# ilia-glushchenko/SimplePathTracer

Measured on AMD Instinct MI355X. Metric: Msamples/s (pixels×spp/s), RTIOW random-sphere scene, 1/2/4/8 MI355X, higher is better.
Workload: dtype f32

## Files before the change

simplepathtracer_amd/csrc/spt_kernels.hip:

```cpp
#include "spt_path.h"
#include "spt_decode.h"

#include <algorithm>
#include <mutex>

namespace spt {


#ifndef SPT_WAVES_PER_EU
#define SPT_WAVES_PER_EU 0
#endif
#ifndef SPT_NUM_SGPR
#define SPT_NUM_SGPR 96
#endif
#if SPT_WAVES_PER_EU
#define SPT_RENDER_ATTR __attribute__((amdgpu_waves_per_eu(SPT_WAVES_PER_EU, SPT_WAVES_PER_EU)))
#elif SPT_NUM_SGPR
#define SPT_CAP_WAVES (800 / (((SPT_NUM_SGPR - 2 + 15) / 16) * 16 + 16) > 8 ? 8 : 800 / (((SPT_NUM_SGPR - 2 + 15) / 16) * 16 + 16))
#define SPT_RENDER_ATTR __attribute__((amdgpu_num_sgpr(SPT_NUM_SGPR), amdgpu_waves_per_eu(SPT_CAP_WAVES)))
#else
#define SPT_RENDER_ATTR
#endif

#ifndef SPT_LDS_BLOCK
// ... 308 lines not shown
                    acc.z = acc.z + c[i].z;
                    if constexpr (!TAB) acc.w = acc.w + 1.f;
                }
            }
            if constexpr (TAB) acc.w = acc.w + (float)kFoldRun;
        }
        for (; k < S; ++k) {
            uint32_t w;
            if constexpr (TAB) {
                w = *ps;
                ps += stp;
            } else {
                w = samples[q0 + k * step];
            }
            const f3 c = decode_word<TAB>(a, w);
            acc.x = acc.x + c.x;
            acc.y = acc.y + c.y;
            acc.z = acc.z + c.z;
            acc.w = acc.w + 1.f;
        }
    } else if (!alias) {
        const uint2 *s2 = (const uint2 *)samples;
        for (uint32_t k = 0; k < S; ++k) {
            const uint2 v = s2[q0 + k * step];
            if (v.y != 0u) {
                const f3 c = decode_word<TAB>(a, v.x);
                acc.x = acc.x + c.x;
                acc.y = acc.y + c.y;
                acc.z = acc.z + c.z;
                acc.w = acc.w + 1.f;
            }
        }
    } else {
        alias_accumulate<TAB>(a, samples, p, W, rows, 0u, rows, S, acc);
    }
    if (!a.last) {
        a.acc[p] = acc;
        if (!a.preview) return;
    }
    const float scale = a.mode == 0 ? 1.f / (float)a.s_done : 1.f / acc.w;
    const float r = acc.x * scale, g = acc.y * scale, b = acc.z * scale;
    if (out_rgba) out_rgba[p] = make_float4(r, g, b, 0.f);
    if (out_rgb8) {
        const uint32_t x = map.x0 + col;
        const uint32_t y = row_of(map, lr);
        const size_t gi = (size_t)3 * ((size_t)(a.height - 1u - y) * a.width + x);
        out_rgb8[gi + 0] = gamma_byte(r);
        out_rgb8[gi + 1] = gamma_byte(g);
        out_rgb8[gi + 2] = gamma_byte(b);
    }
}

#ifndef SPT_SVC_WT
#define SPT_SVC_WT 1
#endif

__device__ __forceinline__ void svc_flush(uint32_t idx, uint32_t cnt, uint32_t lane)
{
    if (cnt == 0u) return;
    kargs_t &k = *kernarg_args();
    asm volatile("s_waitcnt vmcnt(0)" ::: "memory");
    if (!SPT_SVC_WT) {
        __builtin_amdgcn_fence(__ATOMIC_RELEASE, "agent");
        asm volatile("s_waitcnt vmcnt(0)" ::: "memory");
    }
    if (lane == 0) __hip_atomic_fetch_add((gu32 *)(k.svc_done + idx), cnt, __ATOMIC_RELAXED, __HIP_MEMORY_SCOPE_AGENT);
    if (k.svc_trace && lane == 0) atomicMax(k.svc_trace + 4u * idx + 2u, __builtin_amdgcn_s_memrealtime());
}

template <bool TREE, int LEAF, bool LDSN, uint32_t BLOCK, bool BATCH = false, bool GLANE = false, bool SVC = false>
__device__ __forceinline__ void render_body(const RenderArgs &a)
{
    static_assert(!SVC || (!GLANE && !BATCH && (LDSN || SPT_PRIM)),
                  "the render service runs the wave-walk kernel or the LDS lane walk");
    const uint32_t lane = __lane_id();
    const uint32_t rows = SVC ? 0u : a.npix / a.map.width;

    __shared__ uint32_t s_lds[BLOCK];
    __shared__ uint4 s_nodes[LDSN ? 2 * (SVC ? kLdsSvcNodeRecords : kLdsNodeRecords) : 1];
    constexpr bool LDS_BYTES = LDSN && SPT_LANE_WALK && SPT_LANE_BUDGET > 0;
    constexpr bool PRIM = SPT_PRIM && !LDSN && !GLANE;
    constexpr uint32_t PW = kParkWords + (SVC ? 1u : 0u);
    __shared__ uint32_t s_park[PRIM ? (BLOCK / 64u) * PW * 64u : 1];
    uint32_t *const park = s_park + (PRIM ? opaque_v((threadIdx.x >> 6) * PW * 64u + lane) : 0u);
    auto prow = [&](uint32_t r) -> int32_t { return (int32_t)r - (int32_t)lane; };
    __shared__ uint32_t s_rec[SVC ? (BLOCK / 64u) * kSvcRecWords : 1];
    uint32_t *const rec = s_rec + (SVC ? (threadIdx.x >> 6) * kSvcRecWords : 0u);
    if (SVC && lane < kSvcRecWords - kSvcSt) rec[kSvcSt + lane] = 0u;
    if (SVC && !LDSN && blockIdx.x == 0u && (threadIdx.x >> 6) == 0u) {
        svc_forward(lane);
        return;
    }
    uint32_t q_n = 0, q_pos = 0;
    if (LDSN) {
        const uint4 *src = (const uint4 *)a.scene.accel.nodes;
        const uint32_t n4 = 2u * (a.scene.accel.n_nodes + 1u);
        for (uint32_t k = threadIdx.x; k < n4; k += BLOCK) {
            uint4 v = src[k];
            if (LDS_BYTES && (k & 1u)) v.x <<= 5;
            s_nodes[k] = v;
        }
        __syncthreads();
        if (SVC && blockIdx.x == 0u && (threadIdx.x >> 6) == 0u) {
            svc_forward(lane);
            return;
        }
    }
    Path ps;
    ps.phase = PH_IDLE;
    ps.item = ps.bounce = ps.spec = 0;
    ps.st = 0;
    ps.o = ps.d = mk(0.f, 0.f, 0.f);
    ps.slot = 0;
    ps.job = 0;

    uint32_t blk_cur = 0, blk_end = 0;
    uint32_t pend = 0;
    uint32_t rect = 0;
    const uint32_t home = blockIdx.x % a.n_queues;
    uint32_t qi = 0;
    if (SVC)
        pend = svc_reserve(home, lane, 0u);
    else if (lane == 0)
        pend = claim_next(a, home, qi);
    bool exhausted = false;
    uint32_t acc_idx = 0, acc_cnt = 0;
    unsigned long long casts = 0, done = 0, dropped = 0;
    struct {
        unsigned long long iters = 0, cast = 0, shade = 0, refill = 0;
        unsigned long long p_iters = 0, p_nodes = 0, p_spheres = 0, p_branches = 0, p_cast = 0;
        unsigned long long s_rounds[3] = {0, 0, 0};
        unsigned long long t_iters = 0, t_live = 0;
    } dc;
    CastDiag dg;
    Hit hres;
    hres.idx = kMiss;
    hres.best = FLT_MAX;
    hres.t = 0.f;
    uint32_t li = 0, lleaf = kNoSlot, lleaf2 = kNoSlot;
    bool fresh = true;
#if SPT_DIAG
    unsigned long long d_t0 = __builtin_amdgcn_s_memtime();
#define SPT_STAMP(acc)                                              \
    do {                                                            \
        const unsigned long long t_ = __builtin_amdgcn_s_memtime(); \
        acc += t_ - d_t0;                                           \
        d_t0 = t_;                                                  \
    } while (0)
#else
#define SPT_STAMP(acc) \
    do {               \
    } while (0)
#endif

    auto take_items = [&](unsigned long long need) -> uint32_t {
        const uint32_t cnt = (uint32_t)__popcll(need);
        const uint32_t rank = lane_rank(need);
        const uint32_t avail = blk_end - blk_cur;
        uint32_t mine = 0xFFFFFFFFu;
        if (rank < avail) mine = blk_cur + rank;
        if (avail >= cnt) {
            blk_cur += cnt;
        } else {
            const uint32_t nb = __builtin_amdgcn_readfirstlane(pend);
            if (nb < a.n_items && lane == 0) pend = claim_next(a, home, qi);
            if (nb >= a.n_items) {
                exhausted = true;
                blk_cur = blk_end = 0;
            } else {
                const uint32_t ne = min(nb + a.claim, a.n_items);
                const uint32_t r2 = rank - avail;
                if (rank >= avail && r2 < ne - nb) mine = nb + r2;
                blk_cur = nb + min(cnt - avail, ne - nb);
                blk_end = ne;
            }
        }
        return __builtin_amdgcn_inverse_ballot_w64(need) ? mine : 0xFFFFFFFFu;
    };

    auto next_claim = [&]() {
        const uint32_t nb = __builtin_amdgcn_readfirstlane(pend);
        if (nb < a.n_items && lane == 0) pend = claim_next(a, home, qi);
        if (nb >= a.n_items) {
            exhausted = true;
        } else {
            blk_cur = nb;
            blk_end = min(nb + a.claim, a.n_items);
            rect = find_rect(nb);
        }
    };

    auto next_claim_svc = [&]() {
        uint32_t *const st = rec + kSvcSt;
        const uint32_t nb = __builtin_amdgcn_readfirstlane(pend) * a.n_queues + home;
        uint32_t pc = __builtin_amdgcn_readfirstlane(st[0]);
        if (nb >= pc) {
            const unsigned long long p = svc_pub();
            pc = __builtin_amdgcn_readfirstlane((uint32_t)p);
            const uint32_t pj = __builtin_amdgcn_readfirstlane((uint32_t)(p >> 32));
            if (lane == 0) {
                st[0] = pc;
                st[1] = pj;
            }
        }
        exhausted = nb >= pc;
        if (exhausted) return;
        pend = svc_reserve(home, lane, pend);
        if (nb >= __builtin_amdgcn_readfirstlane(st[3])) {
            const uint32_t cur = svc_find_job(nb, __builtin_amdgcn_readfirstlane(st[2]),
                                              __builtin_amdgcn_readfirstlane(st[1]), rec, lane);
            const uint32_t ce = __builtin_amdgcn_readfirstlane(rec[7]);
            if (lane == 0) {
                st[2] = cur;
                st[3] = ce;
            }
        }
        blk_cur = nb * a.claim;
        blk_end = min(blk_cur + a.claim, __builtin_amdgcn_readfirstlane(rec[1]));
        kargs_t &kt = *kernarg_args();
        if (kt.svc_trace && lane == 0) {
            const unsigned long long t = __builtin_amdgcn_s_memrealtime();
            unsigned long long *tr = kt.svc_trace + 4u * rec[3];
            atomicMin(tr, t);
            atomicMax(tr + 1, t);
            if (nb < kSvcTraceClaims)
                kt.svc_trace[4u * 4096u + nb] = (t & 0xFFFFFFFFFFull) | ((unsigned long long)blockIdx.x << 40);
        }
    };

    for (;;) {
        unsigned long long need = __ballot(ps.phase == PH_IDLE);
        if (__popcll(need) < (PRIM ? SPT_PRIM_REFILL_MIN : SPT_REFILL_MIN) && need != ~0ull) need = 0ull;
        bool prim_iter = false;
        uint32_t pxy = 0;
        if (PRIM) {
            if (need != 0ull) {
                const uint32_t cnt = (uint32_t)__popcll(need);
                const uint32_t rank = lane_rank(need);
                const uint32_t take = min(cnt, q_n - q_pos);
                if (ps.phase == PH_IDLE && rank < take) unpark_path<SVC>(park, prow(q_pos + rank), ps);
                q_pos += take;
                bool more = !exhausted;
                if (SVC && cnt > take) {
                    if (blk_cur == blk_end) next_claim_svc();
                    more = blk_cur < blk_end;
                }
                if (cnt > take && more) {
                    park_path<SVC>(park, 0, ps);
                    asm volatile("" ::: "memory");
                    ps.phase = PH_IDLE;
                    if (SVC) {
                        const uint32_t n = min(64u, blk_end - blk_cur);
                        const uint32_t mine = blk_cur + lane;
                        blk_cur += n;
                        if (lane < n) start_path_svc(mine, rec, ps, &pxy);
                    } else if (BATCH) {
                        if (blk_cur == blk_end) next_claim();
                        if (!exhausted) {
                            const uint32_t n = min(64u, blk_end - blk_cur);
                            const uint32_t mine = blk_cur + lane;
                            blk_cur += n;
                            if (lane < n) start_path_rect(mine, rect, ps, &pxy);
                        }
                    } else {
                        const uint32_t mine = take_items(~0ull);
                        if (mine != 0xFFFFFFFFu) start_path_kernarg(mine, rows, ps, &pxy);
                        if ((SPT_DUP & 4) && mine != 0xFFFFFFFFu) {
                            Path p2;
                            uint32_t pxy2 = 0;
                            start_path_kernarg(opaque_v(mine), rows, p2, &pxy2);
                            sink_v(p2.d.x);
                            sink_v(p2.d.y);
                            sink_v(p2.d.z);
                            sink_v(p2.st);
                            sink_v(pxy2);
                        }
                    }
                    prim_iter = true;
                }
            }
        } else if (SVC && !PRIM && need != 0ull) {
            if (blk_cur == blk_end) next_claim_svc();
            if (blk_cur < blk_end) {
                const uint32_t take = min((uint32_t)__popcll(need), blk_end - blk_cur);
                const uint32_t rank = lane_rank(need);
                if (__builtin_amdgcn_inverse_ballot_w64(need) && rank < take) start_path_svc(blk_cur + rank, rec, ps);
                blk_cur += take;
            }
        } else if (BATCH && need != 0ull && !exhausted) {
            if (blk_cur == blk_end) next_claim();
            if (!exhausted) {
                const uint32_t take = min((uint32_t)__popcll(need), blk_end - blk_cur);
                const uint32_t rank = lane_rank(need);
                const uint32_t mine = blk_cur + rank;
                blk_cur += take;
                if (ps.phase == PH_IDLE && rank < take) {
                    start_path_rect(mine, rect, ps);
                }
            }
        } else if (!BATCH && need != 0ull && !exhausted) {
            const uint32_t mine = take_items(need);
            if (mine != 0xFFFFFFFFu) start_path_kernarg(mine, rows, ps);
        }
        const unsigned long long live = __ballot(ps.phase != PH_IDLE);
        if (live == 0ull) {
            if (PRIM && prim_iter) {
                unpark_path<SVC>(park, 0, ps);
                q_n = q_pos = 0;
                continue;
            }
            if (SVC && q_pos == q_n) {
                svc_flush(acc_idx, acc_cnt, lane);
                acc_cnt = 0;
                unsigned long long t0 = __builtin_amdgcn_s_memrealtime();
                bool leave = false;
                bool closing = false;
                uint32_t committed = 0;
                for (;;) {
                    const bool stop = svc_stopped();
                    if (stop) {
                        asm volatile("s_waitcnt vmcnt(0)" ::: "memory");
                        __builtin_amdgcn_fence(__ATOMIC_ACQUIRE, "agent");
                    }
                    if (closing) {
                        kargs_t &k = *kernarg_args();
                        const uint32_t c = lane == 0 ? __hip_atomic_load((gu32 *)(k.svc_host + kSvcHostCommitted),
                                                                         __ATOMIC_SEQ_CST, __HIP_MEMORY_SCOPE_SYSTEM)
                                                     : 0u;
                        asm volatile("s_waitcnt vmcnt(0)" ::: "memory");
                        __builtin_amdgcn_fence(__ATOMIC_ACQUIRE, "agent");
                        committed = __builtin_amdgcn_readfirstlane(c);
                    }
                    next_claim_svc();
                    if (!exhausted) break;
                    if (stop) {
                        leave = true;
                        break;
                    }
                    if (closing) {
                        if (__builtin_amdgcn_readfirstlane(rec[kSvcSt + 1]) >= committed) {
                            kargs_t &k = *kernarg_args();
                            if (lane == 0)
                                __hip_atomic_store((gu32 *)(k.svc_host + kSvcHostWatchdog), 1u, __ATOMIC_RELAXED,
                                                   __HIP_MEMORY_SCOPE_SYSTEM);
                            leave = true;
                            break;
                        }
                        closing = false;
                        t0 = __builtin_amdgcn_s_memrealtime();
                    } else if (__builtin_amdgcn_s_memrealtime() - t0 > kSvcIdleTicks) {
                        kargs_t &k = *kernarg_args();
                        if (lane == 0)
                            __hip_atomic_store((gu32 *)(k.svc_host + kSvcHostClosing), 1u, __ATOMIC_SEQ_CST,
                                               __HIP_MEMORY_SCOPE_SYSTEM);
                        asm volatile("s_waitcnt vmcnt(0)" ::: "memory");
                        __builtin_amdgcn_fence(__ATOMIC_SEQ_CST, "");
                        closing = true;
                        continue;
                    }
                    __builtin_amdgcn_s_sleep(8);
                }
                if (leave) break;
                continue;
            }
            if (exhausted && q_pos == q_n) break;
            continue;
        }
        SPT_STAMP(dc.refill);
#if SPT_DIAG
        const unsigned long long d_n0 = dg.nodes, d_s0 = dg.spheres, d_b0 = dg.branches, d_c0 = dc.cast;
#endif
        constexpr bool RES = SPT_LANE_BUDGET > 0 && (LDSN || GLANE);
        if (!RES) casts += (unsigned long long)__popcll(live);
        ++dc.iters;
        if (SPT_DIAG && exhausted) {
            dc.t_iters += 1;
            dc.t_live += (unsigned long long)__popcll(live);
        }
        const bool act = ps.phase != PH_IDLE;
        bool cdone = true;
        Hit h;
        if constexpr (RES) {
            if (SPT_DUP & 512) {
                Hit h2 = hres;
                h2.best = opaque_v(h2.best);
                uint32_t li2 = opaque_v(li), ll2 = lleaf, ll22 = lleaf2;
                const bool c2 = lane_cast<LEAF, LDS_BYTES>(a.scene.accel, opaque_v3(ps.o), opaque_v3(ps.d), act, dg,
                                    LDSN ? (const uint32_t *)s_nodes : (const uint32_t *)a.scene.accel.nodes, fresh,
                                    (uint32_t)SPT_LANE_BUDGET, h2, li2, ll2, ll22);
                sink_v(h2.idx);
                sink_v(h2.best);
                sink_v(li2);
                sink_v(c2 ? 1u : 0u);
            }
            cdone = lane_cast<LEAF, LDS_BYTES>(a.scene.accel, ps.o, ps.d, act, dg,
                                    LDSN ? (const uint32_t *)s_nodes : (const uint32_t *)a.scene.accel.nodes, fresh,
                                    (uint32_t)SPT_LANE_BUDGET, hres, li, lleaf, lleaf2);
            h = hres;
            casts += (unsigned long long)__popcll(__ballot(act && cdone));
        } else if constexpr (PRIM) {
            bool listed = false;
            if (prim_iter && kernarg_args()->prim.on) {
                if (SPT_DUP & 64) {
                    Hit h2;
                    prim_list_cast(a.scene.accel, opaque_v3(ps.o), opaque_v3(ps.d), act, pxy, h2, dg);
                    sink_v(h2.idx);
                    sink_v(h2.best);
                    sink_v(h2.t);
                }
                listed = prim_list_cast(a.scene.accel, ps.o, ps.d, act, pxy, h, dg);
            }
            if (!listed)
                h = find_closest<TREE, LEAF, LDSN>(a.scene.accel, ps.o, ps.d, act, dg, (const uint32_t *)s_nodes,
                                                   s_lds + (threadIdx.x & ~63u));
            if (SPT_DUP & 1) {
                const f3 o2 = opaque_v3(ps.o), d2 = opaque_v3(ps.d);
                Hit h2;
                bool l2 = false;
                if (prim_iter && kernarg_args()->prim.on) l2 = prim_list_cast(a.scene.accel, o2, d2, act, pxy, h2, dg);
                if (!l2) h2 = find_closest<TREE, LEAF, LDSN>(a.scene.accel, o2, d2, act, dg, (const uint32_t *)s_nodes);
                sink_v(h2.idx);
                sink_v(h2.best);
                sink_v(h2.t);
            }
        } else {
            h = (LDSN && SPT_LANE_WALK)
                    ? find_closest_lane<LEAF>(a.scene.accel, ps.o, ps.d, act, dg, (const uint32_t *)s_nodes)
                : GLANE
                    ? find_closest_lane<LEAF>(a.scene.accel, ps.o, ps.d, act, dg, (const uint32_t *)a.scene.accel.nodes)
                    : find_closest<TREE, LEAF, LDSN>(a.scene.accel, ps.o, ps.d, act, dg, (const uint32_t *)s_nodes);
        }
        SPT_STAMP(dc.cast);
#if SPT_DIAG
        if (prim_iter) {
            dc.p_iters += 1;
            dc.p_nodes += dg.nodes - d_n0;
            dc.p_spheres += dg.spheres - d_s0;
            dc.p_branches += dg.branches - d_b0;
            dc.p_cast += dc.cast - d_c0;
        }
#endif
        shade_step<true, SVC && SPT_SVC_WT>(a, ps, h, act && cdone, done, dropped, s_lds + (threadIdx.x & ~63u),
                                            SPT_DIAG ? dc.s_rounds : nullptr);
        fresh = cdone;
        if (SVC) {
            const bool fin = act && ps.phase == PH_IDLE;
            unsigned long long fm = __ballot(fin);
            while (fm != 0ull) {
                const uint32_t j = __builtin_amdgcn_readlane(ps.job, (int)__builtin_ctzll(fm));
                const unsigned long long m = __ballot(fin && ps.job == j);
                if (j != acc_idx) {
                    svc_flush(acc_idx, acc_cnt, lane);
                    acc_idx = j;
                    acc_cnt = 0;
                }
                acc_cnt += (uint32_t)__popcll(m);
                fm &= ~m;
            }
        }
        if (PRIM && prim_iter) {
            Path own;
            unpark_path<SVC>(park, 0, own);
            __builtin_amdgcn_wave_barrier();
            const unsigned long long lv = __ballot(ps.phase != PH_IDLE);
            if (ps.phase != PH_IDLE) park_path<SVC>(park, prow(lane_rank(lv)), ps);
            ps = own;
            q_n = (uint32_t)__popcll(lv);
            q_pos = 0;
        }
        SPT_STAMP(dc.shade);
    }

    if (SVC) {
        svc_flush(acc_idx, acc_cnt, lane);
        kargs_t &k = *kernarg_args();
        if (lane == 0) __hip_atomic_fetch_add((gu32 *)(k.svc_ctl + kSvcLive), 0xFFFFFFFFu, __ATOMIC_RELAXED, __HIP_MEMORY_SCOPE_AGENT);
    }
#pragma unroll
    for (int o = 32; o > 0; o >>= 1) {
        done += __shfl_xor(done, o);
        dropped += __shfl_xor(dropped, o);
    }
    if (lane == 0) {
        if (casts) atomicAdd(&a.counters[0], casts);
        if (done) atomicAdd(&a.counters[1], done);
        if (dropped) atomicAdd(&a.counters[2], dropped);
    }
#if SPT_DIAG
    if (lane == 0) {
        atomicAdd(&a.counters[4], dc.iters);
        atomicAdd(&a.counters[5], dg.leaves);
        atomicAdd(&a.counters[6], dg.nodes);
        atomicAdd(&a.counters[7], dc.cast);
        atomicAdd(&a.counters[8], dc.shade);
        atomicAdd(&a.counters[9], dc.refill);
        atomicAdd(&a.counters[10], dg.pairs);
        atomicAdd(&a.counters[11], dg.live);
        atomicAdd(&a.counters[12], dg.spheres);
        atomicAdd(&a.counters[13], dg.branches);
        atomicAdd(&a.counters[14], dg.passing);
        atomicAdd(&a.counters[15], dg.improving);
        atomicAdd(&a.counters[16], dg.lane_tests);
        atomicAdd(&a.counters[17], dg.lane_pretests);
        atomicAdd(&a.counters[18], dc.p_iters);
        atomicAdd(&a.counters[19], dc.p_nodes);
        atomicAdd(&a.counters[20], dc.p_spheres);
        atomicAdd(&a.counters[21], dc.p_branches);
        atomicAdd(&a.counters[22], dc.p_cast);
        atomicAdd(&a.counters[23], dc.s_rounds[0]);
        atomicAdd(&a.counters[24], dc.s_rounds[1]);
        atomicAdd(&a.counters[25], dg.leaves8);
        atomicAdd(&a.counters[26], dg.leaves16);
        atomicAdd(&a.counters[27], dc.s_rounds[2]);
        atomicAdd(&a.counters[28], dc.t_iters);
        atomicAdd(&a.counters[29], dc.t_live);
    }
#endif
#undef SPT_STAMP
}

template <bool TREE, int LEAF>
__global__ __launch_bounds__(kRenderBlock) SPT_RENDER_ATTR void render_kernel(RenderArgs a)
{
    render_body<TREE, LEAF, false, kRenderBlock>(a);
}

template <bool TREE, int LEAF>
__global__ __launch_bounds__(kRenderBlock) SPT_RENDER_ATTR void render_kernel_batch(RenderArgs a)
{
    render_body<TREE, LEAF, false, kRenderBlock, true>(a);
}

template <bool TREE, int LEAF>
__global__ __launch_bounds__(kRenderBlock) SPT_RENDER_ATTR void render_kernel_svc(RenderArgs a)
{
    render_body<TREE, LEAF, false, kRenderBlock, false, false, true>(a);
}

__global__ __launch_bounds__(kRenderBlock) SPT_RENDER_ATTR void render_kernel_glane(RenderArgs a)
{
    render_body<true, (int)kClusterSlots, false, kRenderBlock, false, true>(a);
}
__global__ __launch_bounds__(kRenderBlock) SPT_RENDER_ATTR void render_kernel_glane_batch(RenderArgs a)
{
    render_body<true, (int)kClusterSlots, false, kRenderBlock, true, true>(a);
}

#ifndef SPT_LDS_NUM_SGPR
#define SPT_LDS_NUM_SGPR 80
#endif
__global__ __launch_bounds__(kLdsBlock)
    __attribute__((amdgpu_num_sgpr(SPT_LDS_NUM_SGPR), amdgpu_waves_per_eu(2 * kLdsBlock / 256))) void render_kernel_lds(RenderArgs a)
{
    render_body<true, (int)kClusterSlots, true, kLdsBlock>(a);
}
__global__ __launch_bounds__(kLdsBlock)
    __attribute__((amdgpu_num_sgpr(SPT_LDS_NUM_SGPR), amdgpu_waves_per_eu(2 * kLdsBlock / 256))) void render_kernel_lds_batch(RenderArgs a)
{
    render_body<true, (int)kClusterSlots, true, kLdsBlock, true>(a);
}

__global__ __launch_bounds__(kLdsBlock)
    __attribute__((amdgpu_num_sgpr(SPT_LDS_NUM_SGPR), amdgpu_waves_per_eu(2 * kLdsBlock / 256))) void render_kernel_svc_lds(RenderArgs a)
{
    render_body<true, (int)kClusterSlots, true, kLdsBlock, false, false, true>(a);
}

#ifndef SPT_FOLD_PRIO
#define SPT_FOLD_PRIO 3
#endif
// ... 298 lines not shown
```

simplepathtracer_amd/csrc/spt_path.h:

```cpp
#pragma once
#include "spt_device.h"
#include "spt_internal.h"

#include <float.h>

#ifndef SPT_GROUP
#define SPT_GROUP 4
#endif

#ifndef SPT_DIAG
#define SPT_DIAG 0
#endif
#ifndef SPT_LEAF_SPLIT
#define SPT_LEAF_SPLIT 1
#endif
#ifndef SPT_DUP
#define SPT_DUP 0
#endif
#ifndef SPT_SAMPLER_SKIP0
#define SPT_SAMPLER_SKIP0 1
#endif
#ifndef SPT_SAMPLER_EVEN
#define SPT_SAMPLER_EVEN 1
#endif
// ... 909 lines not shown
    const uint32_t bw = k.prim.bw;
    const uint32_t x = pxy & 0xFFFFu, y = pxy >> 16;
    const float dod = dot(o, d);
    cfloat *slots = (cfloat *)ac.slots;
    cuint *ids = (cuint *)k.prim.slots;
    if (SPT_DIAG) dg.live_now = (uint32_t)__popcll(live);
    auto test_run = [&](uint2 e) {
        for (uint32_t i = e.x; i < e.x + e.y; i += 4u) {
            uint32_t s[4];
            float4 sp[4];
#pragma unroll
            for (int q = 0; q < 4; ++q) s[q] = ids[i + q];
#pragma unroll
            for (int q = 0; q < 4; ++q) sp[q] = ld_uniform(slots, s[q]);
            float tcv[4], hv[4];
            bool pass[4];
#pragma unroll
            for (int q = 0; q < 4; ++q) pass[q] = ray_sphere(sp[q], o, d, tcv[q], hv[q]);
            if (SPT_DIAG) dg.lane_tests += 4ull * dg.live_now;
#pragma unroll
            for (int q = 0; q < 4; ++q) {
                const unsigned long long pm = __ballot(pass[q]);
                if (SPT_DIAG) {
                    dg.spheres += 1;
                    dg.branches += pm != 0ull ? 1 : 0;
                }
                if (pm != 0ull) update_member(pm, tcv[q], hv[q], ac.orig, s[q], o, d, dod, h, dg);
            }
        }
    };
    const uint32_t b8 = (y >> 3) * bw + (x >> 3);
    const uint32_t lead = __builtin_amdgcn_readlane(b8, (int)__builtin_ctzll(live));
    if (__ballot(active && b8 != lead) == 0ull) {
        cuint *blk = (cuint *)k.prim.b8 + 2u * lead;
        const uint2 e = make_uint2(blk[0], blk[1]);
        if (e.y == kPrimWalk) return false;
        test_run(e);
        return true;
    }
    const uint32_t b4 = (y >> 2) * bw + (x >> 3);
    unsigned long long todo = live;
    while (todo != 0ull) {
        const uint32_t b = __builtin_amdgcn_readlane(b4, (int)__builtin_ctzll(todo));
        cuint *blk = (cuint *)k.prim.b4 + 2u * b;
        const uint2 e = make_uint2(blk[0], blk[1]);
        if (e.y == kPrimWalk) return false;
        test_run(e);
        todo &= ~__ballot(active && b4 == b);
    }
    return true;
}

__device__ __forceinline__ void refract_event(const float4 *__restrict__ slots, Path &ps, uint32_t idx)
{
    const float4 cs = slots[idx];
    const f3 C = mk(cs.x, cs.y, cs.z);
    const f3 nrm = normalize(sub(ps.o, C));
    const f3 d = ps.d;
    const float cc = dot(neg(nrm), d);
    f3 nd;
    if (uniform(ps.st, 0.f, 1.f) < schlick(kRsq, cc)) {
        nd = reflect(d, nrm);
    } else if (no_tir(kAirToGlass, cc)) {
        const f3 d2 = refract_dir(d, nrm, kAirToGlass, cc);
        const f3 rs = sub(C, ps.o);
        const float tc = dot(rs, d2);
        const float dd = lensq(rs) - tc * tc;
        const float t = tc + __builtin_sqrtf(cs.w - dd);
        ps.o = mk(ps.o.x + d2.x * t, ps.o.y + d2.y * t, ps.o.z + d2.z * t);
        const f3 n2 = neg(normalize(sub(ps.o, C)));
        const float c2 = dot(neg(n2), d2);
        if (uniform(ps.st, 0.f, 1.f) < schlick(kRsq, c2))
            nd = reflect(d2, n2);
        else if (no_tir(kGlassToAir, c2))
            nd = refract_dir(d2, n2, kGlassToAir, c2);
        else
            nd = reflect(d2, n2);
    } else {
        nd = reflect(d, nrm);
    }
    ps.d = nd;
}

template <bool WT = false>
__device__ __forceinline__ void finish_step(uint32_t mode, uint32_t *samples, Path &ps, unsigned long long finm,
                                            unsigned long long specm, unsigned long long refrm, unsigned long long skym,
                                            uint32_t word, unsigned long long &done, unsigned long long &dropped)
{
    typedef __attribute__((address_space(1))) uint32_t gu32_t;
    typedef __attribute__((address_space(1))) unsigned long long gu64_t;
    const uint32_t k = ps.spec & 0xFFFFu;
    const bool spec_event = __builtin_amdgcn_inverse_ballot_w64(specm);
    if (mode == 0u) {
        ps.spec += spec_event ? 1u : 0u;
        const unsigned long long capm = specm & __ballot(k + 1u > kSpecularCap);
        word = __builtin_amdgcn_inverse_ballot_w64(capm) ? kZeroWord : word;
        if (__builtin_amdgcn_inverse_ballot_w64(finm | capm)) {
            if (WT)
                __hip_atomic_store((gu32_t *)(samples + ps.item), word, __ATOMIC_RELAXED, __HIP_MEMORY_SCOPE_AGENT);
            else
                samples[ps.item] = word;
            ps.phase = PH_IDLE;
            ps.d = mk(0.f, 0.f, 0.f);
            ++done;
        }
        return;
    }
    bool fin = __builtin_amdgcn_inverse_ballot_w64(finm);
    const bool refr_event = __builtin_amdgcn_inverse_ballot_w64(refrm), sky = __builtin_amdgcn_inverse_ballot_w64(skym);
    bool counted = true;
    if (spec_event) {
        if (mode == 1u && k < kTaskPasses && refr_event) ps.spec |= 1u << (16u + k);
        ++ps.spec;
        if (mode == 1u && k + 1u >= kTaskPasses) {
            fin = true;
            counted = false;
            word = kZeroWord;
            ++dropped;
        } else if (k + 1u > kSpecularCap) {
            fin = true;
            word = kZeroWord;
        }
    }
    if (fin) {
        const uint32_t key =
            counted ? 1u + (((ps.spec & 0xFFFFu) << 11) | (sky ? 1u << 10 : 0u) | ((ps.spec >> 16) & 0x3FFu)) : 0u;
        if (WT)
            __hip_atomic_store((gu64_t *)(samples + (size_t)2 * ps.item), (unsigned long long)word | ((unsigned long long)key << 32),
                               __ATOMIC_RELAXED, __HIP_MEMORY_SCOPE_AGENT);
        else
            *(uint2 *)(samples + (size_t)2 * ps.item) = make_uint2(word, key);
        ps.phase = PH_IDLE;
        ps.d = mk(0.f, 0.f, 0.f);
        ++done;
    }
}

template <bool KARG, bool WT, bool SAMPLER>
__device__ __forceinline__ void shade_step_body(const RenderArgs &a, Path &ps, const Hit &h, bool act,
                                                unsigned long long &done, unsigned long long &dropped, uint32_t *lds,
                                                unsigned long long *diag_rounds)
{
    const float4 *__restrict__ hit = a.scene.accel.slots;
    const float4 *__restrict__ shade = a.scene.shade;
    const uint32_t *__restrict__ mat = a.scene.mat;
    uint32_t *samples = a.samples;
    uint32_t mode = a.mode;
    uint32_t bounces = a.bounces, code_stride = a.scene.code_stride, code_jmax = a.scene.code_jmax;
    if constexpr (KARG) {
        kargs_t &k = *kernarg_args();
        hit = k.scene.accel.slots;
        shade = k.scene.shade;
        mat = k.scene.mat;
        samples = k.samples;
        mode = k.mode;
        bounces = k.bounces;
        code_stride = k.scene.code_stride;
        code_jmax = k.scene.code_jmax;
    }
    const uint32_t idx = h.idx;
    const unsigned long long actm = __ballot(act);
    const unsigned long long hitm = actm & __ballot(idx != kMiss);
    uint32_t m = SPT_SKYBOX_ID;
    if (__builtin_amdgcn_inverse_ballot_w64(hitm)) m = mat[idx];
    const unsigned long long dlm = actm & __ballot(ps.phase == PH_DLOOP);
    const bool dl = __builtin_amdgcn_inverse_ballot_w64(dlm);
    const uint32_t nb = ps.bounce - 1u;
    ps.bounce = dl ? nb : ps.bounce;
    const unsigned long long endm = dlm & (__ballot(nb == 0u) | ~hitm);
    const unsigned long long trm = actm & ~dlm;
    const unsigned long long diffm = trm & __ballot(m == SPT_DIFFUSE_ID);
    const unsigned long long mirm = trm & __ballot(m == SPT_REFLECTIVE_ID);
    const unsigned long long refrm = trm & __ballot(m == SPT_REFRACTIVE_ID);
    const unsigned long long skym = trm & ~(diffm | mirm | refrm);
    const unsigned long long scatm = (dlm & ~endm) | diffm | mirm;
    const uint32_t j = min(bounces - nb - 1u, code_jmax);
    uint32_t word = kZeroWord;
    word = __builtin_amdgcn_inverse_ballot_w64(endm) ? code_word(diffuse_code(j, ps.slot, code_stride)) : word;
    word = __builtin_amdgcn_inverse_ballot_w64(skym) ? __float_as_uint(ps.d.y + 1.f) : word;
    const f3 rv_coop = SAMPLER ? coop_ball_vector(ps.st, scatm, lds, diag_rounds) : opaque_v3(mk(0.1f, 0.2f, 0.3f));
    if ((SPT_DUP & 2) && SAMPLER) {
        uint64_t st2 = opaque_v(ps.st);
        const bool scatter = __builtin_amdgcn_inverse_ballot_w64(scatm);
        const f3 r2 = coop_ball_vector(st2, __ballot(opaque_v(scatter ? 1u : 0u) != 0u), lds);
        sink_v(r2.x);
        sink_v(r2.y);
        sink_v(r2.z);
        sink_v(st2);
    }
    if (__builtin_amdgcn_inverse_ballot_w64(scatm)) {
        const float4 cs = hit[idx];
        const f3 C = mk(cs.x, cs.y, cs.z);
        ps.o = contact(ps.o, ps.d, h.t);
        const f3 nrm = normalize(sub(ps.o, C));
        f3 rv = rv_coop;
        const f3 on = add(ps.o, nrm);
        f3 base = mk(dl ? on.x : nrm.x, dl ? on.y : nrm.y, dl ? on.z : nrm.z);
        if (__builtin_amdgcn_inverse_ballot_w64(mirm)) {
            base = reflect(ps.d, nrm);
            rv = mul(rv, shade[idx].w);
        }
        ps.d = normalize(add(base, rv));
    }
    const bool first = __builtin_amdgcn_inverse_ballot_w64(diffm);
    ps.slot = first ? idx : ps.slot;
    ps.phase = first ? PH_DLOOP : ps.phase;
    if (__builtin_amdgcn_inverse_ballot_w64(refrm)) {
        ps.o = contact(ps.o, ps.d, h.t);
        if (SPT_DUP & 256) {
            Path p2 = ps;
            p2.o = opaque_v3(p2.o);
            refract_event(hit, p2, idx);
            sink_v(p2.d.x);
            sink_v(p2.o.x);
            sink_v(p2.st);
        }
        refract_event(hit, ps, idx);
    }
    finish_step<WT>(mode, samples, ps, endm | skym, mirm | refrm, refrm, trm, word, done, dropped);
}
template <bool KARG = false, bool WT = false>
__device__ __forceinline__ void shade_step(const RenderArgs &a, Path &ps, const Hit &h, bool act,
                                           unsigned long long &done, unsigned long long &dropped, uint32_t *lds,
                                           unsigned long long *diag_rounds = nullptr)
{
    if (SPT_DUP & 128) {
        Path p2 = ps;
        p2.o = opaque_v3(p2.o);
        p2.d = opaque_v3(p2.d);
        Hit h2 = h;
        h2.t = opaque_v(h2.t);
        unsigned long long d2 = 0, x2 = 0;
        shade_step_body<KARG, WT, false>(a, p2, h2, act, d2, x2, lds, nullptr);
        sink_v(p2.o.x);
        sink_v(p2.d.x);
        sink_v(p2.st);
    }
    shade_step_body<KARG, WT, true>(a, ps, h, act, done, dropped, lds, diag_rounds);
}



__device__ __forceinline__ void start_path(const RenderArgs &a, uint32_t mine, uint32_t rows, const Recip &rw,
                                           const Recip &rh, const f3 &eye, Path &ps, uint32_t *pxy = nullptr)
{
    uint32_t sl, lr, cx;
    ts_item(mine, a.map.width, rows, a.spp_batch, a.div_band, a.div_tile, sl, lr, cx);
    const uint32_t s = a.s0 + sl;
    ps.item = mine;
    const uint32_t x = a.map.x0 + cx;
    const uint32_t y = a.map.parts == 1u ? a.map.y0 + lr : row_of_fast(a.map, lr, a.div_strip);
    if (pxy) *pxy = (y << 16) | x;
    ps.st = fmix64(a.seed_key ^ (((uint64_t)(y * a.width + x) << 32) | (uint64_t)s));
    const float un = (float)y + uniform(ps.st, -1.f, 1.f);
    const float vn = (float)x + uniform(ps.st, -1.f, 1.f);
    float u = div_core(un, rw), v = div_core(vn, rh);
    if (__builtin_expect(!(div_operand_ok(un) && div_operand_ok(vn)), 0)) {
        u = un / (float)a.width;
        v = vn / (float)a.height;
    }
    const float vx = -1.f + 2.f * v, vy = -1.f + 2.f * u;
    const float *m = a.cam.view;
    ps.d = normalize(mk((m[0] * vx + m[1] * vy) + (m[2] * 1.f + m[3] * 0.f),
                        (m[4] * vx + m[5] * vy) + (m[6] * 1.f + m[7] * 0.f),
                        (m[8] * vx + m[9] * vy) + (m[10] * 1.f + m[11] * 0.f)));
    ps.o = eye;
    ps.phase = PH_TRACE;
    ps.bounce = a.bounces;
    ps.spec = 0;
}

__device__ __forceinline__ void start_path_kernarg(uint32_t mine, uint32_t rows, Path &ps, uint32_t *pxy = nullptr)
{
    kargs_t &k = *kernarg_args();
    RenderArgs a;
    a.map = RowMap{k.map.y0, k.map.y1, k.map.strip, k.map.parts, k.map.part, k.map.x0, k.map.width};
    a.width = k.width;
    a.height = k.height;
    a.bounces = k.bounces;
    a.npix = k.npix;
    a.n_items = k.n_items;
    a.spp_batch = k.spp_batch;
    a.s0 = k.s0;
    a.seed_key = k.seed_key;
    a.div_band = FastDiv{k.div_band.d, k.div_band.m, k.div_band.s};
    a.div_tile = FastDiv{k.div_tile.d, k.div_tile.m, k.div_tile.s};
    a.div_strip = FastDiv{k.div_strip.d, k.div_strip.m, k.div_strip.s};
#pragma unroll
    for (int q = 0; q < 12; ++q) a.cam.view[q] = k.cam.view[q];
    start_path(a, mine, rows, recip((float)a.width), recip((float)a.height),
               mk(k.cam.eye[0], k.cam.eye[1], k.cam.eye[2]), ps, pxy);
}

typedef __attribute__((address_space(4))) const BatchRect crect_t;
__device__ __forceinline__ uint32_t find_rect(uint32_t nb)
{
    kargs_t &k = *kernarg_args();
    crect_t *r = k.inline_rects ? (crect_t *)k.rects_inline : (crect_t *)k.rects;
    uint32_t lo = 0, hi = k.n_rects;
    while (hi - lo > 1u) {
        const uint32_t mid = (lo + hi) >> 1;
        if (r[mid].item_off <= nb) lo = mid; else hi = mid;
    }
    return lo;
}

__device__ __forceinline__ void start_path_rect(uint32_t mine, uint32_t ri, Path &ps, uint32_t *pxy = nullptr)
{
    kargs_t &k = *kernarg_args();
    crect_t &r = (k.inline_rects ? (crect_t *)k.rects_inline : (crect_t *)k.rects)[ri];
    if (mine >= r.item_end) return;
    RenderArgs a;
    a.map = RowMap{r.y0, r.y0 + r.rows, 1u, 1u, 0u, r.x0, r.w};
    a.width = k.width;
    a.height = k.height;
// ... 42 lines not shown
```

simplepathtracer_amd/csrc/spt_trace.hip:

```cpp
#include "spt_query.h"
#include "spt_decode.h"

namespace spt {

namespace {

constexpr uint32_t kTraceLaunchRays = 1u << 28;

template <bool TREE, int LEAF, int WALK, uint32_t BLOCK>
__device__ __forceinline__ void trace_body(const TraceArgs &a)
{
    constexpr bool AHEAD = WALK != kWalkLds;
    __shared__ uint32_t s_lds[BLOCK];
    const AccelView &ac = a.scene.accel;
    const uint32_t *const nodes = lds_node_table<WALK, BLOCK>(ac);
    RenderArgs ra;
    ra.scene = a.scene;
    ra.bounces = a.bounces;
    ra.mode = 0u;
    ra.samples = (uint32_t *)a.rgba;
    uint32_t *const lds = s_lds + (threadIdx.x & ~63u);

    const uint32_t lane = __lane_id();
    const uint32_t wave = __builtin_amdgcn_readfirstlane(blockIdx.x * (BLOCK / 64u) + (threadIdx.x >> 6));
    const uint32_t n_waves = gridDim.x * (BLOCK / 64u);
    const uint32_t runs = (a.n + 63u) >> 6;
    uint32_t run = wave, q_n = 0, q_pos = 0;
    f3 qo = mk(0.f, 0.f, 0.f), qd = mk(0.f, 0.f, 0.f);
    uint32_t qs_lo = 0, qs_hi = 0;
    auto load_run = [&]() {
        q_n = run < runs ? min(64u, a.n - (run << 6)) : 0u;
        q_pos = 0;
        if (AHEAD && lane < q_n) {
            const uint32_t i = (run << 6) + lane;
            const float4 o4 = a.o[i], d4 = a.d[i];
            const uint64_t st = a.st[i];
            qo = mk(o4.x, o4.y, o4.z);
            qd = mk(d4.x, d4.y, d4.z);
            qs_lo = (uint32_t)st;
            qs_hi = (uint32_t)(st >> 32);
        }
    };
    load_run();

    Path ps;
    ps.phase = PH_IDLE;
    ps.item = ps.bounce = ps.spec = 0;
    ps.st = 0;
    ps.o = ps.d = mk(0.f, 0.f, 0.f);
    ps.slot = 0;
    ps.job = 0;
    uint32_t casts = 0;
    unsigned long long done = 0, dropped = 0;
    CastDiag dg;

    for (;;) {
        const unsigned long long need = __ballot(ps.phase == PH_IDLE);
        if (need != 0ull && q_n != 0u) {
            const uint32_t take = min((uint32_t)__popcll(need), q_n - q_pos);
            const uint32_t rank = lane_rank(need);
            const bool get = __builtin_amdgcn_inverse_ballot_w64(need) && rank < take;
            const int from = (int)(get ? q_pos + rank : lane);
            f3 o = mk(0.f, 0.f, 0.f), d = o;
            uint64_t st = 0;
            if (AHEAD) {
                o = mk(__shfl(qo.x, from), __shfl(qo.y, from), __shfl(qo.z, from));
                d = mk(__shfl(qd.x, from), __shfl(qd.y, from), __shfl(qd.z, from));
                st = ((uint64_t)(uint32_t)__shfl((int)qs_hi, from) << 32) | (uint32_t)__shfl((int)qs_lo, from);
            }
            if (get) {
                const uint32_t i = (run << 6) + (uint32_t)from;
                if (!AHEAD) {
                    const float4 o4 = a.o[i], d4 = a.d[i];
                    st = a.st[i];
                    o = mk(o4.x, o4.y, o4.z);
                    d = mk(d4.x, d4.y, d4.z);
                }
                ps.o = o;
                ps.d = d;
                ps.st = st;
                ps.item = 4u * i;
                ps.phase = PH_TRACE;
                ps.bounce = a.bounces;
                ps.spec = 0;
                casts = 0;
            }
            q_pos += take;
            if (q_pos == q_n) {
                run += n_waves;
                load_run();
            }
        }
        const unsigned long long live = __ballot(ps.phase != PH_IDLE);
        if (live == 0ull) {
            if (q_n == 0u) break;
            continue;
        }
        const bool act = ps.phase != PH_IDLE;
        const Hit h = query_cast<TREE, LEAF, WALK>(ac, ps.o, ps.d, act, dg, nodes, lds);
        casts += act ? 1u : 0u;
        shade_step(ra, ps, h, act, done, dropped, lds);
        if (act && ps.phase == PH_IDLE && a.info) {
            const uint32_t ev = ps.spec & 0xFFFFu;
            uint32_t *rec = a.info + (ps.item >> 1);
            rec[0] = casts;
            rec[1] = ev | (ev > kSpecularCap ? 0x80000000u : 0u);
        }
    }
}

constexpr uint32_t kTraceBlock = 256, kTraceLdsBlock = 1024;

}

template <bool TREE, int LEAF>
__global__ __launch_bounds__(kTraceBlock) __attribute__((amdgpu_waves_per_eu(6))) void trace_kernel(TraceArgs a)
{
    trace_body<TREE, LEAF, kWalkWave, kTraceBlock>(a);
}
__global__ __launch_bounds__(kTraceBlock) void trace_kernel_glane(TraceArgs a)
{
    trace_body<true, (int)kClusterSlots, kWalkGlane, kTraceBlock>(a);
}
__global__ __launch_bounds__(kTraceLdsBlock) __attribute__((amdgpu_waves_per_eu(2 * kTraceLdsBlock / 256))) void trace_kernel_lds(TraceArgs a)
{
    trace_body<true, (int)kClusterSlots, kWalkLds, kTraceLdsBlock>(a);
}

template <bool TAB>
__global__ __launch_bounds__(256) void trace_decode_kernel(FoldArgs f, float4 *rgba, uint32_t n)
{
    const uint32_t i = blockIdx.x * 256u + threadIdx.x;
    if (i >= n) return;
    const f3 c = decode_word<TAB>(f, f.samples[4u * i]);
    rgba[i] = make_float4(c.x, c.y, c.z, 0.f);
}
// ... 25 lines not shown
```

simplepathtracer_amd/csrc/spt_wavefront.hip:

```cpp
#include "spt_path.h"

#include <algorithm>
#include <mutex>

namespace spt {

namespace {

constexpr uint32_t kWfBlock = 256;
constexpr uint32_t kWfWaves = kWfBlock / 64;

struct WfQueue {
    float4 *o, *d;
    uint4 *m;
};

struct WfArgs {
    RenderArgs ra;
    WfQueue q;
    uint32_t *state;
    uint32_t qcap;
};

__device__ __forceinline__ void load_ray(const WfQueue &q, uint32_t i, Path &ps)
{
    const float4 o = q.o[i], d = q.d[i];
    const uint4 m = q.m[i];
    ps.o = mk(o.x, o.y, o.z);
    ps.slot = __float_as_uint(o.w);
    ps.d = mk(d.x, d.y, d.z);
    ps.item = __float_as_uint(d.w);
    ps.st = (uint64_t)m.x | ((uint64_t)m.y << 32);
    ps.bounce = m.z;
    ps.phase = m.w & 3u;
    ps.spec = m.w >> 2;
}

__device__ __forceinline__ void store_ray(const WfQueue &q, uint32_t i, const Path &ps)
{
    q.o[i] = make_float4(ps.o.x, ps.o.y, ps.o.z, __uint_as_float(ps.slot));
    q.d[i] = make_float4(ps.d.x, ps.d.y, ps.d.z, __uint_as_float(ps.item));
    q.m[i] = make_uint4((uint32_t)ps.st, (uint32_t)(ps.st >> 32), ps.bounce, ps.phase | (ps.spec << 2));
}

template <bool TREE, int LEAF, bool GLANE>
__global__ __launch_bounds__(kWfBlock) void wf_render(WfArgs w)
{
    __shared__ float4 s_o[kWfBlock], s_d[kWfBlock];
    __shared__ uint4 s_m[kWfBlock];
    __shared__ float2 s_h[kWfBlock];
    __shared__ uint32_t s_lds[kWfBlock];
    __shared__ uint32_t s_cnt[kWfWaves][kWfCats + 1];
    __shared__ uint32_t s_claim;

    typedef __attribute__((address_space(1))) uint32_t gu32;
    const RenderArgs &a = w.ra;
    const uint32_t tid = threadIdx.x, wave = tid >> 6, lane = __lane_id();
    const uint32_t rows = a.npix / a.map.width;
    const Recip rw = recip((float)a.width), rh = recip((float)a.height);
    const f3 eye = mk(a.cam.eye[0], a.cam.eye[1], a.cam.eye[2]);
    const size_t q0 = (size_t)blockIdx.x * w.qcap;
    const WfQueue q{w.q.o + q0, w.q.d + q0, w.q.m + q0};
    uint32_t len = 0;
    unsigned long long cast = 0, finished = 0, done = 0, dropped = 0;
    for (;;) {
        if (tid == 0) s_claim = __hip_atomic_fetch_add((gu32 *)w.state, w.qcap - len, __ATOMIC_RELAXED, __HIP_MEMORY_SCOPE_AGENT);
        __syncthreads();
        const uint32_t first = s_claim;
        const uint32_t got = first < a.n_items ? min(w.qcap - len, a.n_items - first) : 0u;
        const uint32_t n = len + got;
        if (n == 0u) break;
        uint32_t wp = 0;
        for (uint32_t base = 0; base < n; base += kWfBlock) {
            const uint32_t i = base + tid;
            const uint32_t live = min(n - base, kWfBlock);
            const bool act = i < n;
            Path ps;
            ps.phase = PH_IDLE;
            ps.item = ps.bounce = ps.spec = ps.slot = 0;
            ps.st = 0;
            ps.o = ps.d = mk(0.f, 0.f, 0.f);
            if (act) {
                if (i < len) {
                    load_ray(q, i, ps);
                } else {
                    start_path(a, first + (i - len), rows, rw, rh, eye, ps);
                    ps.slot = 0;
                }
            }
            CastDiag dg;
            const Hit h = GLANE ? find_closest_lane<LEAF>(a.scene.accel, ps.o, ps.d, act, dg, (const uint32_t *)a.scene.accel.nodes)
                                : find_closest<TREE, LEAF>(a.scene.accel, ps.o, ps.d, act, dg);
            uint32_t cat = kWfCats;
            if (act) {
                cat = 0u;
                if (ps.phase == PH_DLOOP) {
                    cat = 4u;
                } else if (h.idx != kMiss) {
                    const uint32_t mt = a.scene.mat[h.idx];
                    cat = mt == SPT_DIFFUSE_ID ? 1u : mt == SPT_REFLECTIVE_ID ? 2u : mt == SPT_REFRACTIVE_ID ? 3u : 0u;
                }
            }
            uint32_t rank = 0;
#pragma unroll
            for (uint32_t c = 0; c < kWfCats; ++c) {
                const unsigned long long m = __ballot(cat == c);
                if (lane == 0) s_cnt[wave][c] = (uint32_t)__popcll(m);
                if (cat == c) rank = lane_rank(m);
            }
            __syncthreads();
            if (act) {
                uint32_t pos = rank;
#pragma unroll
                for (uint32_t c = 0; c < kWfCats; ++c)
#pragma unroll
                    for (uint32_t v = 0; v < kWfWaves; ++v)
                        if (c < cat || (c == cat && v < wave)) pos += s_cnt[v][c];
                s_o[pos] = make_float4(ps.o.x, ps.o.y, ps.o.z, __uint_as_float(ps.slot));
                s_d[pos] = make_float4(ps.d.x, ps.d.y, ps.d.z, __uint_as_float(ps.item));
                s_m[pos] = make_uint4((uint32_t)ps.st, (uint32_t)(ps.st >> 32), ps.bounce, ps.phase | (ps.spec << 2));
                s_h[pos] = make_float2(h.t, __uint_as_float(h.idx));
            }
            __syncthreads();
            const bool act2 = tid < live;
            Hit hh;
            hh.best = 0.f;
            hh.t = 0.f;
            hh.idx = kMiss;
            if (act2) {
                const float4 o = s_o[tid], d = s_d[tid];
                const uint4 m = s_m[tid];
                const float2 t = s_h[tid];
                ps.o = mk(o.x, o.y, o.z);
                ps.slot = __float_as_uint(o.w);
                ps.d = mk(d.x, d.y, d.z);
                ps.item = __float_as_uint(d.w);
                ps.st = (uint64_t)m.x | ((uint64_t)m.y << 32);
                ps.bounce = m.z;
                ps.phase = m.w & 3u;
                ps.spec = m.w >> 2;
                hh.t = t.x;
                hh.idx = __float_as_uint(t.y);
            } else {
                ps.phase = PH_IDLE;
            }
            shade_step(a, ps, hh, act2, done, dropped, s_lds + wave * 64u);
            const bool alive = act2 && ps.phase != PH_IDLE;
            const unsigned long long am = __ballot(alive);
            if (lane == 0) s_cnt[wave][kWfCats] = (uint32_t)__popcll(am);
            __syncthreads();
            uint32_t at = wp + lane_rank(am), tot = 0;
#pragma unroll
            for (uint32_t v = 0; v < kWfWaves; ++v) {
                const uint32_t k = s_cnt[v][kWfCats];
                if (v < wave) at += k;
                tot += k;
            }
            if (alive) store_ray(q, at, ps);
            wp += tot;
            __syncthreads();
        }
        cast += n;
        finished += n - wp;
        len = wp;
    }
    (void)done;
    if (tid == 0) {
        atomicAdd(&a.counters[0], cast);
        atomicAdd(&a.counters[1], finished);
    }
    if (dropped) atomicAdd(&a.counters[2], dropped);
}

template <bool TREE, int LEAF, bool GLANE>
uint32_t resident_blocks(int dev)
{
    static std::mutex mu;
    static int cached[64];
    std::lock_guard<std::mutex> lk(mu);
    if (dev < 0 || dev >= 64) return 0;
    if (cached[dev] == 0) {
        int per_cu = 0, cus = 0;
        if (hipOccupancyMaxActiveBlocksPerMultiprocessor(&per_cu, wf_render<TREE, LEAF, GLANE>, kWfBlock, 0) != hipSuccess ||
            hipDeviceGetAttribute(&cus, hipDeviceAttributeMultiprocessorCount, dev) != hipSuccess)
            return 0;
        cached[dev] = std::max(per_cu, 0) * std::max(cus, 0);
        if (cached[dev] == 0) cached[dev] = -1;
    }
    return cached[dev] > 0 ? (uint32_t)cached[dev] : 0u;
}

template <bool TREE, int LEAF, bool GLANE>
hipError_t launch(const WavefrontBuffers &b, const RenderArgs &a, hipStream_t s)
{
    int dev = 0;
    hipError_t e = hipGetDevice(&dev);
    if (e != hipSuccess) return e;
    const uint32_t resident = resident_blocks<TREE, LEAF, GLANE>(dev);
    if (resident == 0) return hipErrorInvalidConfiguration;
    const uint32_t grid = std::max(1u, std::min(resident, b.cap / b.qcap));
    WfArgs w;
    w.ra = a;
    w.q = WfQueue{b.o, b.d, b.m};
    w.state = b.state;
    w.qcap = b.qcap;
    e = hipMemsetAsync(b.state, 0, kWfStateWords * sizeof(uint32_t), s);
    if (e != hipSuccess) return e;
    hipLaunchKernelGGL((wf_render<TREE, LEAF, GLANE>), dim3(grid), dim3(kWfBlock), 0, s, w);
    return hipGetLastError();
}

}

uint32_t wavefront_blocks(const AccelView &ac, int dev)
{
    if (lane_walk_tree(ac)) return resident_blocks<true, (int)kClusterSlots, true>(dev);
    if (ac.tree) return resident_blocks<true, (int)kClusterSlots, false>(dev);
    if (ac.leaf_slots == kFlatLeafSlots) return resident_blocks<false, (int)kFlatLeafSlots, false>(dev);
    return resident_blocks<false, (int)kClusterSlots, false>(dev);
}

hipError_t launch_wavefront(const WavefrontBuffers &b, const RenderArgs &a, hipStream_t s)
{
    if (a.n_items == 0) return hipSuccess;
    if (lane_walk_tree(a.scene.accel)) return launch<true, (int)kClusterSlots, true>(b, a, s);
    if (a.scene.accel.tree) return launch<true, (int)kClusterSlots, false>(b, a, s);
    if (a.scene.accel.leaf_slots == kFlatLeafSlots) return launch<false, (int)kFlatLeafSlots, false>(b, a, s);
    return launch<false, (int)kClusterSlots, false>(b, a, s);
}

}
```

Before: 26280.

## Park only live paths in LDS with wave-uniform base and ballot-based counters

Replaces the per-lane park layout (opaque per-lane offset, always park own path then re-park survivors after shading) with a wave-uniform LDS base where only live paths are compacted by rank at refill time, removing the post-shade unpark/repark pass. The done/dropped counters become 32-bit wave-uniform counts accumulated via ballot popcount instead of per-lane 64-bit increments plus a final shuffle reduction, and flushing is folded into a helper called at service flush points. This is meant to cut LDS traffic, VGPR pressure and reduction work, but it changes when parked paths are restored and risks counter overflow or double counting if the ballots cover inactive lanes.

```diff
diff --git a/simplepathtracer_amd/csrc/spt_kernels.hip b/simplepathtracer_amd/csrc/spt_kernels.hip
--- a/simplepathtracer_amd/csrc/spt_kernels.hip
+++ b/simplepathtracer_amd/csrc/spt_kernels.hip
@@ -414,8 +414,8 @@
     constexpr bool PRIM = SPT_PRIM && !LDSN && !GLANE;
     constexpr uint32_t PW = kParkWords + (SVC ? 1u : 0u);
     __shared__ uint32_t s_park[PRIM ? (BLOCK / 64u) * PW * 64u : 1];
-    uint32_t *const park = s_park + (PRIM ? opaque_v((threadIdx.x >> 6) * PW * 64u + lane) : 0u);
-    auto prow = [&](uint32_t r) -> int32_t { return (int32_t)r - (int32_t)lane; };
+    const uint32_t park_base = PRIM ? __builtin_amdgcn_readfirstlane(threadIdx.x & ~63u) * PW : 0u;
+    auto park_rows = [&]() -> uint32_t * { return s_park + park_base; };
     __shared__ uint32_t s_rec[SVC ? (BLOCK / 64u) * kSvcRecWords : 1];
     uint32_t *const rec = s_rec + (SVC ? (threadIdx.x >> 6) * kSvcRecWords : 0u);
     if (SVC && lane < kSvcRecWords - kSvcSt) rec[kSvcSt + lane] = 0u;
@@ -457,7 +457,8 @@
         pend = claim_next(a, home, qi);
     bool exhausted = false;
     uint32_t acc_idx = 0, acc_cnt = 0;
-    unsigned long long casts = 0, done = 0, dropped = 0;
+    unsigned long long casts = 0;
+    uint32_t done = 0, dropped = 0;
     struct {
         unsigned long long iters = 0, cast = 0, shade = 0, refill = 0;
         unsigned long long p_iters = 0, p_nodes = 0, p_spheres = 0, p_branches = 0, p_cast = 0;
@@ -560,6 +561,16 @@
         }
     };
 
+    auto add_counts = [&]() {
+        if (lane == 0) {
+            if (casts) atomicAdd(&a.counters[0], casts);
+            if (done) atomicAdd(&a.counters[1], (unsigned long long)done);
+            if (dropped) atomicAdd(&a.counters[2], (unsigned long long)dropped);
+        }
+        casts = 0;
+        done = dropped = 0;
+    };
+
     for (;;) {
         unsigned long long need = __ballot(ps.phase == PH_IDLE);
         if (__popcll(need) < (PRIM ? SPT_PRIM_REFILL_MIN : SPT_REFILL_MIN) && need != ~0ull) need = 0ull;
@@ -570,7 +581,8 @@
                 const uint32_t cnt = (uint32_t)__popcll(need);
                 const uint32_t rank = lane_rank(need);
                 const uint32_t take = min(cnt, q_n - q_pos);
-                if (ps.phase == PH_IDLE && rank < take) unpark_path<SVC>(park, prow(q_pos + rank), ps);
+                uint32_t *const park = park_rows();
+                if (ps.phase == PH_IDLE && rank < take) unpark_path<SVC>(park, (int32_t)(q_pos + rank), ps);
                 q_pos += take;
                 bool more = !exhausted;
                 if (SVC && cnt > take) {
@@ -578,7 +590,10 @@
                     more = blk_cur < blk_end;
                 }
                 if (cnt > take && more) {
-                    park_path<SVC>(park, 0, ps);
+                    const unsigned long long ownm = __ballot(ps.phase != PH_IDLE);
+                    if (ps.phase != PH_IDLE) park_path<SVC>(park, (int32_t)lane_rank(ownm), ps);
+                    q_pos = 0;
+                    q_n = (uint32_t)__popcll(ownm);
                     asm volatile("" ::: "memory");
                     ps.phase = PH_IDLE;
                     if (SVC) {
@@ -636,14 +651,10 @@
         }
         const unsigned long long live = __ballot(ps.phase != PH_IDLE);
         if (live == 0ull) {
-            if (PRIM && prim_iter) {
-                unpark_path<SVC>(park, 0, ps);
-                q_n = q_pos = 0;
-                continue;
-            }
             if (SVC && q_pos == q_n) {
                 svc_flush(acc_idx, acc_cnt, lane);
                 acc_cnt = 0;
+                add_counts();
                 unsigned long long t0 = __builtin_amdgcn_s_memrealtime();
                 bool leave = false;
                 bool closing = false;
@@ -783,6 +794,7 @@
                 const unsigned long long m = __ballot(fin && ps.job == j);
                 if (j != acc_idx) {
                     svc_flush(acc_idx, acc_cnt, lane);
+                    add_counts();
                     acc_idx = j;
                     acc_cnt = 0;
                 }
@@ -790,16 +802,6 @@
                 fm &= ~m;
             }
         }
-        if (PRIM && prim_iter) {
-            Path own;
-            unpark_path<SVC>(park, 0, own);
-            __builtin_amdgcn_wave_barrier();
-            const unsigned long long lv = __ballot(ps.phase != PH_IDLE);
-            if (ps.phase != PH_IDLE) park_path<SVC>(park, prow(lane_rank(lv)), ps);
-            ps = own;
-            q_n = (uint32_t)__popcll(lv);
-            q_pos = 0;
-        }
         SPT_STAMP(dc.shade);
     }
 
@@ -808,16 +810,7 @@
         kargs_t &k = *kernarg_args();
         if (lane == 0) __hip_atomic_fetch_add((gu32 *)(k.svc_ctl + kSvcLive), 0xFFFFFFFFu, __ATOMIC_RELAXED, __HIP_MEMORY_SCOPE_AGENT);
     }
-#pragma unroll
-    for (int o = 32; o > 0; o >>= 1) {
-        done += __shfl_xor(done, o);
-        dropped += __shfl_xor(dropped, o);
-    }
-    if (lane == 0) {
-        if (casts) atomicAdd(&a.counters[0], casts);
-        if (done) atomicAdd(&a.counters[1], done);
-        if (dropped) atomicAdd(&a.counters[2], dropped);
-    }
+    add_counts();
 #if SPT_DIAG
     if (lane == 0) {
         atomicAdd(&a.counters[4], dc.iters);
diff --git a/simplepathtracer_amd/csrc/spt_path.h b/simplepathtracer_amd/csrc/spt_path.h
--- a/simplepathtracer_amd/csrc/spt_path.h
+++ b/simplepathtracer_amd/csrc/spt_path.h
@@ -1015,10 +1015,10 @@
     ps.d = nd;
 }
 
-template <bool WT = false>
+template <bool WT = false, class CNT>
 __device__ __forceinline__ void finish_step(uint32_t mode, uint32_t *samples, Path &ps, unsigned long long finm,
                                             unsigned long long specm, unsigned long long refrm, unsigned long long skym,
-                                            uint32_t word, unsigned long long &done, unsigned long long &dropped)
+                                            uint32_t word, CNT &done, CNT &dropped)
 {
     typedef __attribute__((address_space(1))) uint32_t gu32_t;
     typedef __attribute__((address_space(1))) unsigned long long gu64_t;
@@ -1028,6 +1028,7 @@
         ps.spec += spec_event ? 1u : 0u;
         const unsigned long long capm = specm & __ballot(k + 1u > kSpecularCap);
         word = __builtin_amdgcn_inverse_ballot_w64(capm) ? kZeroWord : word;
+        done += (CNT)__popcll(finm | capm);
         if (__builtin_amdgcn_inverse_ballot_w64(finm | capm)) {
             if (WT)
                 __hip_atomic_store((gu32_t *)(samples + ps.item), word, __ATOMIC_RELAXED, __HIP_MEMORY_SCOPE_AGENT);
@@ -1035,7 +1036,6 @@
                 samples[ps.item] = word;
             ps.phase = PH_IDLE;
             ps.d = mk(0.f, 0.f, 0.f);
-            ++done;
         }
         return;
     }
@@ -1049,12 +1049,13 @@
             fin = true;
             counted = false;
             word = kZeroWord;
-            ++dropped;
         } else if (k + 1u > kSpecularCap) {
             fin = true;
             word = kZeroWord;
         }
     }
+    dropped += (CNT)__popcll(__ballot(!counted));
+    done += (CNT)__popcll(__ballot(fin));
     if (fin) {
         const uint32_t key =
             counted ? 1u + (((ps.spec & 0xFFFFu) << 11) | (sky ? 1u << 10 : 0u) | ((ps.spec >> 16) & 0x3FFu)) : 0u;
@@ -1065,13 +1066,12 @@
             *(uint2 *)(samples + (size_t)2 * ps.item) = make_uint2(word, key);
         ps.phase = PH_IDLE;
         ps.d = mk(0.f, 0.f, 0.f);
-        ++done;
-    }
-}
-
-template <bool KARG, bool WT, bool SAMPLER>
+    }
+}
+
+template <bool KARG, bool WT, bool SAMPLER, class CNT>
 __device__ __forceinline__ void shade_step_body(const RenderArgs &a, Path &ps, const Hit &h, bool act,
-                                                unsigned long long &done, unsigned long long &dropped, uint32_t *lds,
+                                                CNT &done, CNT &dropped, uint32_t *lds,
                                                 unsigned long long *diag_rounds)
 {
     const float4 *__restrict__ hit = a.scene.accel.slots;
@@ -1152,9 +1152,9 @@
     }
     finish_step<WT>(mode, samples, ps, endm | skym, mirm | refrm, refrm, trm, word, done, dropped);
 }
-template <bool KARG = false, bool WT = false>
+template <bool KARG = false, bool WT = false, class CNT>
 __device__ __forceinline__ void shade_step(const RenderArgs &a, Path &ps, const Hit &h, bool act,
-                                           unsigned long long &done, unsigned long long &dropped, uint32_t *lds,
+                                           CNT &done, CNT &dropped, uint32_t *lds,
                                            unsigned long long *diag_rounds = nullptr)
 {
     if (SPT_DUP & 128) {
@@ -1163,7 +1163,7 @@
         p2.d = opaque_v3(p2.d);
         Hit h2 = h;
         h2.t = opaque_v(h2.t);
-        unsigned long long d2 = 0, x2 = 0;
+        CNT d2 = 0, x2 = 0;
         shade_step_body<KARG, WT, false>(a, p2, h2, act, d2, x2, lds, nullptr);
         sink_v(p2.o.x);
         sink_v(p2.d.x);
diff --git a/simplepathtracer_amd/csrc/spt_trace.hip b/simplepathtracer_amd/csrc/spt_trace.hip
--- a/simplepathtracer_amd/csrc/spt_trace.hip
+++ b/simplepathtracer_amd/csrc/spt_trace.hip
@@ -51,7 +51,7 @@
     ps.slot = 0;
     ps.job = 0;
     uint32_t casts = 0;
-    unsigned long long done = 0, dropped = 0;
+    uint32_t done = 0, dropped = 0;
     CastDiag dg;
 
     for (;;) {
diff --git a/simplepathtracer_amd/csrc/spt_wavefront.hip b/simplepathtracer_amd/csrc/spt_wavefront.hip
--- a/simplepathtracer_amd/csrc/spt_wavefront.hip
+++ b/simplepathtracer_amd/csrc/spt_wavefront.hip
@@ -62,7 +62,8 @@
     const size_t q0 = (size_t)blockIdx.x * w.qcap;
     const WfQueue q{w.q.o + q0, w.q.d + q0, w.q.m + q0};
     uint32_t len = 0;
-    unsigned long long cast = 0, finished = 0, done = 0, dropped = 0;
+    unsigned long long cast = 0, finished = 0;
+    uint32_t done = 0, dropped = 0;
     for (;;) {
         if (tid == 0) s_claim = __hip_atomic_fetch_add((gu32 *)w.state, w.qcap - len, __ATOMIC_RELAXED, __HIP_MEMORY_SCOPE_AGENT);
         __syncthreads();
@@ -169,7 +170,7 @@
         atomicAdd(&a.counters[0], cast);
         atomicAdd(&a.counters[1], finished);
     }
-    if (dropped) atomicAdd(&a.counters[2], dropped);
+    if (lane == 0 && dropped) atomicAdd(&a.counters[2], (unsigned long long)dropped);
 }
 
 template <bool TREE, int LEAF, bool GLANE>
```

New measurement: 28420 (median of 6 runs). 8.2% higher.
